# muzishen/IMAGDressing

Measured on NVIDIA H100. Metric: images/sec, 512x512 50-step DDIM garment-conditioned (CFG), higher is better.
Workload: dtype bf16

## Files before the change

### imagdressing_b200/_lib.py

```python
from __future__ import annotations

import ctypes
import os
from ctypes import POINTER, Structure, c_char_p, c_float, c_int, c_int32, c_int64, c_void_p

_HERE = os.path.dirname(os.path.abspath(__file__))
LIB_PATH = os.path.join(_HERE, "libimagd_b200.so")

IMAGD_OK = 0
ACT_NONE, ACT_GEGLU, ACT_SILU, ACT_GELU, ACT_QUICK_GELU = 0, 1, 2, 3, 4


class Epilogue(Structure):

    _fields_ = [
        ("bias", c_void_p),
        ("rowvec", c_void_p),
        ("rowvec_ld", c_int64),
        ("rows_per_group", c_int32),
        ("act", c_int32),
        ("residual", c_void_p),
        ("ldr", c_int64),
        ("alpha", c_float),
        ("out_fp32", c_int32),
        ("row_stats_out", c_void_p),
        ("stats_ld", c_int64),
        ("row_stats_in", c_void_p),
        ("stats_in_ld", c_int64),
        ("stats_parts", c_int32),
        ("ln_dim", c_int32),
        ("ln_eps", c_float),
        ("colsum", c_void_p),
    ]


class AttnTrain(Structure):

    _fields_ = [("lse", c_void_p), ("out_s0", c_void_p), ("out_s1", c_void_p), ("ld_s", c_int64), ("lq_pad", c_int32)]


class KVStream(Structure):

    _fields_ = [
        ("k", c_void_p),
        ("v", c_void_p),
        ("ld", c_int64),
        ("len", c_int32),
        ("sample_rows", c_int32),
        ("broadcast", c_int32),
        ("n_query_samples", c_int32),
        ("out_scale", c_float),
    ]


SIGNATURES = {
    "imagd_version": (c_int, []),
    "imagd_last_error": (c_char_p, []),
    "imagd_device_check": (c_int, []),
    "imagd_gemm_bf16": (c_int, [c_void_p, c_int64, c_void_p, c_int64, c_void_p, c_int64, c_int, c_int, c_int,
                                POINTER(Epilogue), c_void_p]),
    "imagd_gemm_debug_force": (c_int, [c_int, c_int, c_int]),
    "imagd_gemm_debug_log": (c_int, [c_int, c_char_p, c_int]),
    "imagd_gemm_debug_timeline": (c_int, [c_void_p]),
    "imagd_gemm_tile_count_n": (c_int, [c_int, c_int, c_int]),
    "imagd_conv3x3_bf16": (c_int, [c_void_p, c_int64, c_int, c_int, c_int, c_int, c_void_p, c_void_p, c_int64, c_int,
                                   POINTER(Epilogue), c_void_p]),
    "imagd_upconv3x3_bf16": (c_int, [c_void_p, c_int64, c_int, c_int, c_int, c_int, c_void_p, c_void_p, c_int64, c_int,
                                     POINTER(Epilogue), c_void_p]),
    "imagd_attention_bf16": (c_int, [c_void_p, c_int64, c_void_p, c_int64, c_int, c_int, c_int, c_int,
                                     POINTER(KVStream), POINTER(KVStream), c_float, c_void_p]),
    "imagd_attention_causal_bf16": (c_int, [c_void_p, c_int64, c_void_p, c_int64, c_int, c_int, c_int, c_int,
                                            POINTER(KVStream), c_float, c_void_p]),
    "imagd_groupnorm_ws_bytes": (c_int64, [c_int, c_int, c_int, c_int]),
    "imagd_groupnorm_bf16": (c_int, [c_void_p, c_int64, c_void_p, c_int64, c_int, c_int, c_int, c_int, c_void_p,
                                     c_void_p, c_float, c_int, c_void_p, c_void_p]),
    "imagd_layernorm_bf16": (c_int, [c_void_p, c_int64, c_void_p, c_int64, c_int, c_int, c_void_p, c_void_p, c_float,
                                     c_void_p]),
    "imagd_concat_add_bf16": (c_int, [c_void_p, c_int64, c_int, c_void_p, c_int64, c_void_p, c_int64, c_int, c_void_p,
                                      c_int64, c_void_p, c_int64, c_int64, c_void_p]),
    "imagd_upsample2x_bf16": (c_int, [c_void_p, c_void_p, c_int, c_int, c_int, c_int, c_void_p]),
    "imagd_im2col3x3_s2_bf16": (c_int, [c_void_p, c_void_p, c_int, c_int, c_int, c_int, c_void_p]),
    "imagd_im2col3x3_s2_pad_bf16": (c_int, [c_void_p, c_void_p, c_int, c_int, c_int, c_int, c_int, c_void_p]),
    "imagd_embed_tokens_bf16": (c_int, [c_void_p, c_void_p, c_void_p, c_void_p, c_int, c_int, c_int, c_int, c_void_p]),
    "imagd_patchify_bf16": (c_int, [c_void_p, c_void_p, c_int, c_int, c_int, c_int, c_int, c_void_p]),
    "imagd_broadcast_row_bf16": (c_int, [c_void_p, c_void_p, c_int, c_int64, c_int, c_int, c_void_p]),
    "imagd_softmax_rows": (c_int, [c_void_p, c_int64, c_void_p, c_int64, c_int64, c_int, c_float, c_void_p]),
    "imagd_conv3x3_direct_bf16": (c_int, [c_void_p, c_int, c_int, c_int, c_int, c_void_p, c_void_p, c_void_p, c_int,
                                          c_int, c_int, c_int, c_void_p, c_void_p]),
    "imagd_nchw_f32_to_nhwc_bf16": (c_int, [c_void_p, c_void_p, c_int, c_int, c_int, c_int, c_int, c_int, c_void_p]),
    "imagd_timestep_embedding": (c_int, [c_void_p, c_void_p, c_void_p, c_int, c_int, c_void_p]),
    "imagd_linear_small_m": (c_int, [c_void_p, c_int64, c_void_p, c_int64, c_void_p, c_void_p, c_int64, c_int, c_int,
                                     c_int, c_int, c_int, c_void_p]),
    "imagd_cfg_ddim_step": (c_int, [c_void_p, c_void_p, c_float, c_void_p, c_void_p, c_void_p, c_void_p, c_void_p,
                                    c_void_p, c_void_p, c_int, c_int, c_int, c_void_p]),
    "imagd_nchw_f32_to_nhwc_bf16_scaled": (c_int, [c_void_p, c_void_p, c_int, c_int, c_int, c_int, c_int, c_int, c_void_p,
                                                   c_void_p, c_void_p]),
    "imagd_cfg_sampler_step": (c_int, [c_void_p, c_void_p, c_float, c_void_p, c_void_p, c_void_p, c_void_p, c_void_p,
                                       c_void_p, c_void_p, c_void_p, c_void_p, c_int, c_int, c_int, c_void_p]),
    "imagd_attention_train_fwd_bf16": (c_int, [c_void_p, c_int64, c_void_p, c_int64, c_int, c_int, c_int, c_int,
                                               POINTER(KVStream), POINTER(KVStream), c_float, POINTER(AttnTrain), c_void_p]),
    "imagd_attention_bwd_prep": (c_int, [c_void_p, c_int64, c_void_p, c_void_p, c_int64, c_float, c_float, c_void_p, c_int,
                                         c_int, c_int, c_int, c_int, c_void_p]),
    "imagd_attention_bwd_bf16": (c_int, [c_void_p, c_int64, c_void_p, c_int64, c_int, c_int, c_int, c_int, POINTER(KVStream),
                                         POINTER(KVStream), c_float, c_void_p, c_void_p, c_int, c_void_p, c_int64, c_void_p,
                                         c_void_p, c_int64, c_void_p, c_void_p, c_int64, c_void_p]),
    "imagd_transpose_bf16": (c_int, [c_void_p, c_int64, c_void_p, c_int64, c_int, c_int, c_int, c_void_p]),
    "imagd_conv_weight_layout_bf16": (c_int, [c_void_p, c_void_p, c_int, c_int, c_int, c_void_p]),
    "imagd_conv_weight_flip_bf16": (c_int, [c_void_p, c_void_p, c_int, c_int, c_void_p]),
    "imagd_im2col3x3_t_bf16": (c_int, [c_void_p, c_void_p, c_int64, c_int, c_int, c_int, c_int, c_void_p]),
    "imagd_col2im3x3_s2_bf16": (c_int, [c_void_p, c_void_p, c_int, c_int, c_int, c_int, c_void_p]),
    "imagd_downsum2x_bf16": (c_int, [c_void_p, c_void_p, c_int, c_int, c_int, c_int, c_void_p]),
    "imagd_colreduce_ws_bytes": (c_int64, [c_int, c_int, c_int]),
    "imagd_colsum_bf16": (c_int, [c_void_p, c_int64, c_int, c_int, c_int, c_void_p, c_int, c_void_p, c_void_p]),
    "imagd_layernorm_bwd_bf16": (c_int, [c_void_p, c_int64, c_void_p, c_int64, c_void_p, c_int64, c_int, c_int, c_void_p,
                                         c_float, c_void_p, c_void_p, c_int, c_void_p, c_void_p, c_void_p]),
    "imagd_groupnorm_stats_bf16": (c_int, [c_void_p, c_int64, c_void_p, c_int64, c_int, c_int, c_int, c_int, c_void_p,
                                           c_void_p, c_float, c_int, c_void_p, c_void_p, c_void_p]),
    "imagd_groupnorm_bwd_ws_bytes": (c_int64, [c_int, c_int, c_int, c_int]),
    "imagd_groupnorm_bwd_bf16": (c_int, [c_void_p, c_void_p, c_void_p, c_int, c_int, c_int, c_int, c_void_p, c_void_p,
                                         c_void_p, c_int, c_void_p, c_void_p, c_int, c_void_p, c_void_p]),
    "imagd_act_bf16": (c_int, [c_void_p, c_void_p, c_void_p, c_int64, c_int, c_void_p]),
    "imagd_geglu_bf16": (c_int, [c_void_p, c_int64, c_void_p, c_void_p, c_int64, c_int64, c_int, c_void_p]),
    "imagd_mse_loss_grad": (c_int, [c_void_p, c_void_p, c_void_p, c_void_p, c_int64, c_float, c_void_p, c_void_p]),
    "imagd_adamw_step": (c_int, [c_void_p, c_void_p, c_void_p, c_void_p, c_void_p, c_int64, c_float, c_float, c_float,
                                 c_float, c_float, c_int, c_float, c_void_p]),
    "imagd_adamw_step_dev": (c_int, [c_void_p, c_void_p, c_void_p, c_void_p, c_void_p, c_int64, c_float, c_float, c_float,
# ... 102 lines not shown
```

### imagdressing_b200/csrc/norm.cu

```cuda
#include <cooperative_groups.h>

#include <cstdlib>

#include "common.cuh"
#include "ptx.cuh"

namespace imagd {

constexpr int kGnMaxC = 2560;
constexpr int kGnThreads = 512;
constexpr int kGnCounters = 1024;

static int gn_pixels_per_chunk() {
    static int v = 0;
    if (v == 0) {
        const char* e = getenv("IMAGD_GN_PX");
        v = e ? atoi(e) : 16;
        if (v < 4 || v > 256) v = 16;
    }
    return v;
}
static int gn_max_chunks() {
    static int v = 0;
    if (v == 0) {
        const char* e = getenv("IMAGD_GN_MAXCHUNKS");
        v = e ? atoi(e) : 64;
        if (v < 1 || v > kNumSms) v = 64;
    }
    return v;
}
inline int gn_chunks(int HW, int NB) {
    const int px = gn_pixels_per_chunk();
    int c = (HW + px - 1) / px;
    const int cap = (kNumSms * 2) / (NB > 0 ? NB : 1);
    if (c > gn_max_chunks()) c = gn_max_chunks();
    if (c > cap) c = cap;
    return c < 1 ? 1 : c;
}

__global__ void __launch_bounds__(kGnThreads, 2) groupnorm_fused_kernel(
    const __nv_bfloat16* __restrict__ x, int64_t ldx, __nv_bfloat16* __restrict__ y, int64_t ldy, int HW, int C,
    int groups, int chunks, float* __restrict__ ws, const float* __restrict__ gamma, const float* __restrict__ beta,
    float eps, int fuse_silu, float* __restrict__ stats_out) {
    pdl_launch_dependents();
    pdl_wait();
    __shared__ float s_a[kGnThreads * 8];
    __shared__ float s_b[kGnThreads * 8];
    __shared__ float s_mean[64];
    __shared__ float s_rstd[64];
    extern __shared__ float s_affine[];
    float* s_gamma = s_affine;
    float* s_beta = s_affine + C;
    float* s_piv = s_affine + 2 * C;
    const int n = blockIdx.y, chunk = blockIdx.x;
    const int CV = C / 8;
    const int rows = kGnThreads / CV;
    const int ppc = (HW + chunks - 1) / chunks;
    const int p_begin = chunk * ppc;
    const int p_end = min(HW, p_begin + ppc);
    const int cpg = C / groups;
    for (int c = threadIdx.x; c < C; c += kGnThreads) {
        s_gamma[c] = gamma ? __ldg(gamma + c) : 1.f;
        s_beta[c] = beta ? __ldg(beta + c) : 0.f;
    }
    unsigned int* counters = reinterpret_cast<unsigned int*>(ws) - kGnCounters + 2 * n;

    const int cv = threadIdx.x % CV;
    const int prow = threadIdx.x / CV;
    if (prow < rows) {
        float sum[8], sq[8], piv[8];
#pragma unroll
        for (int k = 0; k < 8; ++k) sum[k] = sq[k] = piv[k] = 0.f;
        const __nv_bfloat16* base = x + (static_cast<int64_t>(n) * HW) * ldx + cv * 8;
        if (p_begin < p_end) {
            const uint4 pv = __ldg(reinterpret_cast<const uint4*>(base + static_cast<int64_t>(p_begin) * ldx));
            const uint32_t u[4] = {pv.x, pv.y, pv.z, pv.w};
#pragma unroll
            for (int k = 0; k < 4; ++k) {
                piv[2 * k] = bf16lo(u[k]);
                piv[2 * k + 1] = bf16hi(u[k]);
            }
        }
        if (prow == 0) {
#pragma unroll
            for (int k = 0; k < 8; ++k) s_piv[cv * 8 + k] = piv[k];
        }
        for (int pix = p_begin + prow; pix < p_end; pix += rows * 4) {
            uint4 v[4];
// ... 108 lines not shown
        }
        __syncthreads();
    }
    for (int c = threadIdx.x; c < C; c += kGnThreads) {
        const int g = c / cpg;
        const float sc = s_gamma[c] * s_rstd[g];
        s_a[c] = sc;
        s_b[c] = s_beta[c] - s_mean[g] * sc;
    }
    __syncthreads();
    const int total = (p_end - p_begin) * CV;
    constexpr int U = 4;
    const int step_row = kGnThreads / CV, step_col = kGnThreads % CV;
    int walk_row = threadIdx.x / CV, walk_col = threadIdx.x % CV;
    for (int base = threadIdx.x; base < total; base += kGnThreads * U) {
        uint4 v[U];
        int c0s[U];
        int64_t rowsv[U];
#pragma unroll
        for (int t = 0; t < U; ++t) {
            const int idx = base + t * kGnThreads;
            v[t] = make_uint4(0u, 0u, 0u, 0u);
            c0s[t] = walk_col * 8;
            rowsv[t] = static_cast<int64_t>(n) * HW + p_begin + walk_row;
            if (idx < total) v[t] = __ldg(reinterpret_cast<const uint4*>(x + rowsv[t] * ldx + c0s[t]));
            walk_row += step_row;
            walk_col += step_col;
            if (walk_col >= CV) {
                walk_col -= CV;
                ++walk_row;
            }
        }
#pragma unroll
        for (int t = 0; t < U; ++t) {
            if (base + t * kGnThreads >= total) break;
            const uint32_t u[4] = {v[t].x, v[t].y, v[t].z, v[t].w};
            const int c0 = c0s[t];
            float f[8];
#pragma unroll
            for (int k = 0; k < 4; ++k) {
                f[2 * k] = bf16lo(u[k]) * s_a[c0 + 2 * k] + s_b[c0 + 2 * k];
                f[2 * k + 1] = bf16hi(u[k]) * s_a[c0 + 2 * k + 1] + s_b[c0 + 2 * k + 1];
            }
            if (fuse_silu) {
#pragma unroll
                for (int k = 0; k < 8; ++k) f[k] = silu(f[k]);
            }
            *reinterpret_cast<uint4*>(y + rowsv[t] * ldy + c0) = make_uint4(
                pack_bf16x2(f[0], f[1]), pack_bf16x2(f[2], f[3]), pack_bf16x2(f[4], f[5]), pack_bf16x2(f[6], f[7]));
        }
    }
}

constexpr int kGnCS = 8;
__global__ void __launch_bounds__(kGnThreads, 2) groupnorm_cluster_kernel(
    const __nv_bfloat16* __restrict__ x, int64_t ldx, __nv_bfloat16* __restrict__ y, int64_t ldy, int HW, int C,
    int groups, int gps, const float* __restrict__ gamma, const float* __restrict__ beta, float eps, int fuse_silu,
    float* __restrict__ stats_out) {
    pdl_launch_dependents();
    pdl_wait();
    namespace cg = cooperative_groups;
    cg::cluster_group cluster = cg::this_cluster();
    __shared__ float s_a[kGnThreads * 8];
    __shared__ float s_b[kGnThreads * 8];
    __shared__ float s_part[64 * 2];
    __shared__ float s_mean[64];
    __shared__ float s_rstd[64];
    extern __shared__ __align__(16) unsigned char s_dyn[];
    const int cpg = C / groups;
    const int SC = gps * cpg;
    const int SV = SC / 8;
    float* s_gamma = reinterpret_cast<float*>(s_dyn);
    float* s_beta = s_gamma + SC;
    float* s_piv = s_beta + SC;
    uint4* tile = reinterpret_cast<uint4*>(s_dyn + ((3 * SC * sizeof(float) + 15) / 16) * 16);
    const int rank = static_cast<int>(cluster.block_rank());
    const int slice = blockIdx.x / kGnCS, n = blockIdx.y;
    const int c_base = slice * SC;
    const int rpc = (HW + kGnCS - 1) / kGnCS;
    const int p_begin = min(HW, rank * rpc);
    const int p_end = min(HW, p_begin + rpc);
    for (int c = threadIdx.x; c < SC; c += kGnThreads) {
        s_gamma[c] = gamma ? __ldg(gamma + c_base + c) : 1.f;
        s_beta[c] = beta ? __ldg(beta + c_base + c) : 0.f;
    }
    const int cv = threadIdx.x % SV;
    const int prow = threadIdx.x / SV;
    const int rows = kGnThreads / SV;
    if (prow < rows) {
        float sum[8], sq[8], piv[8];
#pragma unroll
        for (int k = 0; k < 8; ++k) sum[k] = sq[k] = piv[k] = 0.f;
        const __nv_bfloat16* base = x + (static_cast<int64_t>(n) * HW) * ldx + c_base + cv * 8;
        if (p_begin < p_end) {
            const uint4 pv = __ldg(reinterpret_cast<const uint4*>(base + static_cast<int64_t>(p_begin) * ldx));
            const uint32_t u[4] = {pv.x, pv.y, pv.z, pv.w};
#pragma unroll
            for (int k = 0; k < 4; ++k) {
                piv[2 * k] = bf16lo(u[k]);
                piv[2 * k + 1] = bf16hi(u[k]);
            }
        }
        if (prow == 0) {
#pragma unroll
            for (int k = 0; k < 8; ++k) s_piv[cv * 8 + k] = piv[k];
        }
        for (int pix = p_begin + prow; pix < p_end; pix += rows * 4) {
            uint4 v[4];
            float live[4];
#pragma unroll
            for (int t = 0; t < 4; ++t) {
                v[t] = make_uint4(0u, 0u, 0u, 0u);
                live[t] = 0.f;
                if (pix + t * rows < p_end) {
                    v[t] = __ldg(reinterpret_cast<const uint4*>(base + static_cast<int64_t>(pix + t * rows) * ldx));
                    live[t] = 1.f;
                }
            }
#pragma unroll
            for (int t = 0; t < 4; ++t) {
                if (pix + t * rows < p_end) tile[(pix + t * rows - p_begin) * SV + cv] = v[t];
                const uint32_t u[4] = {v[t].x, v[t].y, v[t].z, v[t].w};
#pragma unroll
                for (int k = 0; k < 4; ++k) {
                    const float a = (bf16lo(u[k]) - piv[2 * k]) * live[t], b = (bf16hi(u[k]) - piv[2 * k + 1]) * live[t];
                    sum[2 * k] += a;
                    sq[2 * k] += a * a;
                    sum[2 * k + 1] += b;
                    sq[2 * k + 1] += b * b;
                }
            }
        }
#pragma unroll
        for (int k = 0; k < 8; ++k) {
            s_a[prow * SC + cv * 8 + k] = sum[k];
            s_b[prow * SC + cv * 8 + k] = sq[k];
        }
    }
    __syncthreads();
    for (int c = threadIdx.x; c < SC; c += kGnThreads) {
        float a = s_a[c], b = s_b[c];
        for (int r = 1; r < rows; ++r) {
            a += s_a[r * SC + c];
            b += s_b[r * SC + c];
        }
        s_a[c] = a;
        s_b[c] = b;
    }
    __syncthreads();
    if (threadIdx.x < gps) {
        const int g = threadIdx.x;
        const float npix = static_cast<float>(p_end - p_begin);
        const float inv = npix > 0.f ? 1.f / npix : 0.f;
        float mean_g = 0.f;
        for (int c = g * cpg; c < (g + 1) * cpg; ++c) mean_g += s_piv[c] + s_a[c] * inv;
        mean_g /= static_cast<float>(cpg);
        float m2 = 0.f;
        for (int c = g * cpg; c < (g + 1) * cpg; ++c) {
            const float d = s_piv[c] + s_a[c] * inv - mean_g;
            m2 += (s_b[c] - s_a[c] * s_a[c] * inv) + npix * d * d;
        }
        s_part[2 * g] = npix > 0.f ? mean_g : 0.f;
        s_part[2 * g + 1] = npix > 0.f ? m2 : 0.f;
    }
    cluster.sync();
    if (threadIdx.x < gps) {
        const int g = threadIdx.x;
        float a = 0.f, b = 0.f;
        const float pivot = cluster.map_shared_rank(s_part, 0)[2 * g];
        for (int r = 0; r < kGnCS; ++r) {
            const float* rp = cluster.map_shared_rank(s_part, r);
            const float cnt_r = static_cast<float>(cpg) * static_cast<float>(max(min(HW, (r + 1) * rpc) - min(HW, r * rpc), 0));
            const float d = rp[2 * g] - pivot;
            a += cnt_r * d;
            b += rp[2 * g + 1] + cnt_r * d * d;
        }
        const float cnt = static_cast<float>(cpg) * static_cast<float>(HW);
        const float dm = a / cnt;
        const float var = fmaxf((b - a * dm) / cnt, 0.f);
        s_mean[g] = pivot + dm;
        s_rstd[g] = rsqrtf(var + eps);
        if (stats_out != nullptr && rank == 0) {
            stats_out[(static_cast<int64_t>(n) * groups + slice * gps + g) * 2] = pivot + dm;
            stats_out[(static_cast<int64_t>(n) * groups + slice * gps + g) * 2 + 1] = s_rstd[g];
        }
    }
    cluster.barrier_arrive();
    __syncthreads();
    for (int c = threadIdx.x; c < SC; c += kGnThreads) {
        const int g = c / cpg;
        const float sc = s_gamma[c] * s_rstd[g];
        s_a[c] = sc;
        s_b[c] = s_beta[c] - s_mean[g] * sc;
    }
    __syncthreads();
    const int total = (p_end - p_begin) * SV;
    const int step_row = kGnThreads / SV, step_col = kGnThreads % SV;
    int walk_row = prow, walk_col = cv;
    for (int idx = threadIdx.x; idx < total; idx += kGnThreads) {
        const uint4 v = tile[idx];
        const int c0 = walk_col * 8;
        const int64_t row = static_cast<int64_t>(n) * HW + p_begin + walk_row;
        walk_row += step_row;
        walk_col += step_col;
        if (walk_col >= SV) {
            walk_col -= SV;
            ++walk_row;
        }
        const uint32_t u[4] = {v.x, v.y, v.z, v.w};
        float f[8];
#pragma unroll
        for (int k = 0; k < 4; ++k) {
            f[2 * k] = bf16lo(u[k]) * s_a[c0 + 2 * k] + s_b[c0 + 2 * k];
            f[2 * k + 1] = bf16hi(u[k]) * s_a[c0 + 2 * k + 1] + s_b[c0 + 2 * k + 1];
        }
        if (fuse_silu) {
#pragma unroll
            for (int k = 0; k < 8; ++k) f[k] = silu(f[k]);
        }
        *reinterpret_cast<uint4*>(y + row * ldy + c_base + c0) = make_uint4(
            pack_bf16x2(f[0], f[1]), pack_bf16x2(f[2], f[3]), pack_bf16x2(f[4], f[5]), pack_bf16x2(f[6], f[7]));
    }
    cluster.barrier_wait();
}

template <int VPL, int R>
__global__ void __launch_bounds__(256) layernorm_kernel(const __nv_bfloat16* __restrict__ x, int64_t ldx,
                                                        __nv_bfloat16* __restrict__ y, int64_t ldy, int rows, int C,
// ... 30 lines not shown
                f[i][2 * k] = bf16lo(u[k]);
                f[i][2 * k + 1] = bf16hi(u[k]);
                sum += f[i][2 * k] + f[i][2 * k + 1];
            }
        }
#pragma unroll
        for (int o = 16; o > 0; o >>= 1) sum += __shfl_xor_sync(0xffffffffu, sum, o);
        const float mean = sum * inv_c;
        float sq = 0.f;
#pragma unroll
        for (int i = 0; i < VPL; ++i) {
            if (lane + i * 32 < CV) {
#pragma unroll
                for (int k = 0; k < 8; ++k) {
                    const float d = f[i][k] - mean;
                    sq += d * d;
                }
            }
        }
#pragma unroll
        for (int o = 16; o > 0; o >>= 1) sq += __shfl_xor_sync(0xffffffffu, sq, o);
        const float rstd = rsqrtf(sq * inv_c + eps);
#pragma unroll
        for (int i = 0; i < VPL; ++i) {
            const int cv = lane + i * 32;
            if (cv < CV) {
                float o[8];
                float g[8], b[8];
                if (gamma) {
                    const float4 g0 = __ldg(reinterpret_cast<const float4*>(gamma + cv * 8));
                    const float4 g1 = __ldg(reinterpret_cast<const float4*>(gamma + cv * 8 + 4));
                    g[0] = g0.x; g[1] = g0.y; g[2] = g0.z; g[3] = g0.w; g[4] = g1.x; g[5] = g1.y; g[6] = g1.z; g[7] = g1.w;
                } else {
#pragma unroll
                    for (int k = 0; k < 8; ++k) g[k] = 1.f;
                }
                if (beta) {
                    const float4 b0 = __ldg(reinterpret_cast<const float4*>(beta + cv * 8));
                    const float4 b1 = __ldg(reinterpret_cast<const float4*>(beta + cv * 8 + 4));
                    b[0] = b0.x; b[1] = b0.y; b[2] = b0.z; b[3] = b0.w; b[4] = b1.x; b[5] = b1.y; b[6] = b1.z; b[7] = b1.w;
                } else {
#pragma unroll
                    for (int k = 0; k < 8; ++k) b[k] = 0.f;
                }
#pragma unroll
                for (int k = 0; k < 8; ++k) o[k] = (f[i][k] - mean) * rstd * g[k] + b[k];
                *reinterpret_cast<uint4*>(y + static_cast<int64_t>(row0 + r) * ldy + cv * 8) =
                    make_uint4(pack_bf16x2(o[0], o[1]), pack_bf16x2(o[2], o[3]), pack_bf16x2(o[4], o[5]), pack_bf16x2(o[6], o[7]));
            }
        }
    }
}

static int gn_cluster_mode() {
    static int v = -1;
    if (v < 0) {
        const char* e = getenv("IMAGD_GN_CLUSTER");
        v = e ? atoi(e) : 1;
        if (v < 0 || v > 2) v = 1;
    }
    return v;
}
struct GnClusterPlan {
    int gps;
    size_t smem;
};
constexpr size_t kGnClusterMaxDyn = 190 * 1024;
static bool gn_cluster_plan(int NB, int HW, int C, int groups, GnClusterPlan* plan) {
    const int mode = gn_cluster_mode();
    if (mode == 0) return false;
    const int cpg = C / groups;
    if (mode == 1 && cpg < 10) return false;
    const int rpc = (HW + kGnCS - 1) / kGnCS;
    double best = 0.0;
    bool found = false;
    for (int gps = 1; gps <= groups; ++gps) {
        if (groups % gps != 0) continue;
        const int SC = gps * cpg;
        if (SC % 8 != 0 || SC / 8 > kGnThreads) continue;
        const size_t tile = static_cast<size_t>(rpc) * SC * 2;
        const size_t dyn = (3 * static_cast<size_t>(SC) * sizeof(float) + 15) / 16 * 16 + tile;
        if (dyn > kGnClusterMaxDyn) continue;
        const int per_sm = (dyn + 35 * 1024) * 2 <= 228 * 1024 ? 2 : 1;
        const int64_t ctas = static_cast<int64_t>(NB) * (groups / gps) * kGnCS;
        const int64_t slots = 144LL * per_sm;
        const int64_t waves = (ctas + slots - 1) / slots;
        if (mode == 1 && (waves > 1 || tile > 32 * 1024)) continue;
        const double cost = static_cast<double>(waves) * (64.0 * 1024 + static_cast<double>(tile) * (SC * 2 < 128 ? 1.3 : 1.0));
        if (!found || cost < best) {
            best = cost;
            plan->gps = gps;
            plan->smem = dyn;
            found = true;
        }
    }
    return found;
}

template <int VPL, int R>
static int launch_ln(const void* x, int64_t ldx, void* y, int64_t ldy, int rows, int C, const float* gamma,
                     const float* beta, float eps, cudaStream_t st) {
    const int rows_per_block = 8 * R;
    IMAGD_CUDA(launch_pdl(layernorm_kernel<VPL, R>, dim3((rows + rows_per_block - 1) / rows_per_block), dim3(256), 0, st,
                          reinterpret_cast<const __nv_bfloat16*>(x), ldx, reinterpret_cast<__nv_bfloat16*>(y), ldy, rows, C,
                          gamma, beta, eps));
    return IMAGD_OK;
}

}

extern "C" {

int64_t imagd_groupnorm_ws_bytes(int NB, int HW, int C, int groups) {
    (void)C;
    return (imagd::kGnCounters + static_cast<int64_t>(NB) * imagd::gn_chunks(HW, NB) * groups * 2) * sizeof(float);
}

int imagd_groupnorm_bf16(const void* x, int64_t ldx, void* y, int64_t ldy, int NB, int HW, int C, int groups,
                         const float* gamma, const float* beta, float eps, int fuse_silu, void* ws, imagd_stream stream) {
    return imagd_groupnorm_stats_bf16(x, ldx, y, ldy, NB, HW, C, groups, gamma, beta, eps, fuse_silu, ws, nullptr, stream);
}

int imagd_groupnorm_stats_bf16(const void* x, int64_t ldx, void* y, int64_t ldy, int NB, int HW, int C, int groups,
                               const float* gamma, const float* beta, float eps, int fuse_silu, void* ws, float* stats_out,
                               imagd_stream stream) {
    using namespace imagd;
    IMAGD_CHECK_ARG(x && y && ws, "groupnorm: null pointer");
    IMAGD_CHECK_ARG(NB > 0 && 2 * NB <= kGnCounters && NB <= kNumSms * 2 && HW > 0 && C > 0 && C % 8 == 0 && C <= kGnMaxC,
                    "groupnorm: NB=%d C=%d unsupported", NB, C);
    IMAGD_CHECK_ARG(groups > 0 && groups <= 64 && C % groups == 0, "groupnorm: groups=%d", groups);
    IMAGD_CHECK_ARG(ldx % 8 == 0 && ldy % 8 == 0 && aligned16(x) && aligned16(y), "groupnorm: alignment");
    cudaStream_t st = static_cast<cudaStream_t>(stream);
    GnClusterPlan plan;
    if (gn_cluster_plan(NB, HW, C, groups, &plan)) {
        IMAGD_SET_MAX_SMEM(groupnorm_cluster_kernel, static_cast<int>(kGnClusterMaxDyn));
        cudaLaunchConfig_t cfg{};
        cfg.gridDim = dim3(kGnCS * (groups / plan.gps), NB);
        cfg.blockDim = dim3(kGnThreads);
        cfg.dynamicSmemBytes = plan.smem;
        cfg.stream = st;
        cudaLaunchAttribute attr[2];
        attr[0].id = cudaLaunchAttributeClusterDimension;
        attr[0].val.clusterDim.x = kGnCS;
        attr[0].val.clusterDim.y = 1;
        attr[0].val.clusterDim.z = 1;
        attr[1].id = cudaLaunchAttributeProgrammaticStreamSerialization;
        attr[1].val.programmaticStreamSerializationAllowed = 1;
        cfg.attrs = attr;
        cfg.numAttrs = pdl_enabled() ? 2 : 1;
        IMAGD_CUDA(cudaLaunchKernelEx(&cfg, groupnorm_cluster_kernel, reinterpret_cast<const __nv_bfloat16*>(x), ldx,
                                      reinterpret_cast<__nv_bfloat16*>(y), ldy, HW, C, groups, plan.gps, gamma, beta, eps,
                                      fuse_silu, stats_out));
        return IMAGD_OK;
    }
    const int chunks = gn_chunks(HW, NB);
    IMAGD_SET_MAX_SMEM(groupnorm_fused_kernel, 64 * 1024);
    IMAGD_CUDA(launch_pdl(groupnorm_fused_kernel, dim3(chunks, NB), dim3(kGnThreads), 3 * C * sizeof(float), st,
                          reinterpret_cast<const __nv_bfloat16*>(x), ldx, reinterpret_cast<__nv_bfloat16*>(y), ldy, HW, C,
                          groups, chunks, reinterpret_cast<float*>(ws) + kGnCounters, gamma, beta, eps, fuse_silu, stats_out));
    return IMAGD_OK;
}

int imagd_layernorm_bf16(const void* x, int64_t ldx, void* y, int64_t ldy, int rows, int C, const float* gamma,
                         const float* beta, float eps, imagd_stream stream) {
    using namespace imagd;
    IMAGD_CHECK_ARG(x && y, "layernorm: null pointer");
    IMAGD_CHECK_ARG(rows > 0 && C > 0 && C % 8 == 0 && C <= 2048, "layernorm: C=%d unsupported", C);
    IMAGD_CHECK_ARG(ldx % 8 == 0 && ldy % 8 == 0 && aligned16(x) && aligned16(y), "layernorm: alignment");
    IMAGD_CHECK_ARG((!gamma || aligned16(gamma)) && (!beta || aligned16(beta)), "layernorm: gamma/beta alignment");
    cudaStream_t st = static_cast<cudaStream_t>(stream);
    const int vpl = (C / 8 + 31) / 32;
    if (vpl <= 2) return launch_ln<2, 4>(x, ldx, y, ldy, rows, C, gamma, beta, eps, st);
    if (vpl <= 3) return launch_ln<3, 4>(x, ldx, y, ldy, rows, C, gamma, beta, eps, st);
    if (vpl <= 5) return launch_ln<5, 2>(x, ldx, y, ldy, rows, C, gamma, beta, eps, st);
    return launch_ln<8, 1>(x, ldx, y, ldy, rows, C, gamma, beta, eps, st);

}

}
```

### include/imagd_b200.h

```cpp
#ifndef IMAGD_B200_H
#define IMAGD_B200_H

#include <stdint.h>

#ifdef __cplusplus
extern "C" {
#endif

typedef void* imagd_stream;

enum imagd_status {
    IMAGD_OK = 0,
    IMAGD_ERR_ARG = -1,
    IMAGD_ERR_CUDA = -2,
    IMAGD_ERR_ARCH = -3
};

enum imagd_act { IMAGD_ACT_NONE = 0, IMAGD_ACT_GEGLU = 1, IMAGD_ACT_SILU = 2, IMAGD_ACT_GELU = 3,
                 IMAGD_ACT_QUICK_GELU = 4  };

int imagd_version(void);
const char* imagd_last_error(void);
int imagd_device_check(void);

// ... 1 lines not shown
    const float* bias;
    const float* rowvec;
    int64_t rowvec_ld;
    int32_t rows_per_group;
    int32_t act;
    const void* residual;
    int64_t ldr;
    float alpha;
    int32_t out_fp32;
    float* row_stats_out;
    int64_t stats_ld;
    const float* row_stats_in;
    int64_t stats_in_ld;
    int32_t stats_parts;
    int32_t ln_dim;
    float ln_eps;
    const float* colsum;
} imagd_epilogue;

int imagd_gemm_bf16(const void* A, int64_t lda, const void* W, int64_t ldw, void* D, int64_t ldd, int M, int N,
                    int K, const imagd_epilogue* ep, imagd_stream stream);

int imagd_gemm_debug_force(int block_n, int stages, int splits);
int imagd_upconv3x3_bf16(const void* X, int64_t ldx, int NB, int H, int W, int Cin, const void* Wt, void* Y, int64_t ldy,
                         int Cout, const imagd_epilogue* ep, imagd_stream stream);
int imagd_gemm_tile_count_n(int M, int N, int K);
int imagd_gemm_debug_log(int enable, char* out, int out_bytes);
int imagd_gemm_debug_timeline(void* device_buf);

int imagd_conv3x3_bf16(const void* X, int64_t ldx, int NB, int H, int W, int Cin, const void* Wt, void* Y,
                       int64_t ldy, int Cout, const imagd_epilogue* ep, imagd_stream stream);

typedef struct imagd_kv_stream {
    const void* k;
    const void* v;
    int64_t ld;
    int32_t len;
    int32_t sample_rows;
    int32_t broadcast;
    int32_t n_query_samples;
    float out_scale;
} imagd_kv_stream;

int imagd_attention_bf16(const void* q, int64_t q_ld, void* out, int64_t out_ld, int B, int Lq, int heads,
                         int head_dim, const imagd_kv_stream* s0, const imagd_kv_stream* s1, float sm_scale,
                         imagd_stream stream);
int imagd_attention_causal_bf16(const void* q, int64_t q_ld, void* out, int64_t out_ld, int B, int Lq, int heads,
                                int head_dim, const imagd_kv_stream* s0, float sm_scale, imagd_stream stream);

int64_t imagd_groupnorm_ws_bytes(int NB, int HW, int C, int groups);
int imagd_groupnorm_bf16(const void* x, int64_t ldx, void* y, int64_t ldy, int NB, int HW, int C, int groups,
                         const float* gamma, const float* beta, float eps, int fuse_silu, void* ws,
                         imagd_stream stream);
int imagd_layernorm_bf16(const void* x, int64_t ldx, void* y, int64_t ldy, int rows, int C, const float* gamma,
                         const float* beta, float eps, imagd_stream stream);

int imagd_concat_add_bf16(const void* a, int64_t lda, int Ca, const void* res_a, int64_t ld_ra, const void* b,
                          int64_t ldb, int Cb, const void* res_b, int64_t ld_rb, void* out, int64_t ldo,
                          int64_t rows, imagd_stream stream);
int imagd_upsample2x_bf16(const void* x, void* y, int NB, int H, int W, int C, imagd_stream stream);
int imagd_im2col3x3_s2_bf16(const void* x, void* col, int NB, int H, int W, int C, imagd_stream stream);
int imagd_im2col3x3_s2_pad_bf16(const void* x, void* col, int NB, int H, int W, int C, int pad_lo, imagd_stream stream);
int imagd_softmax_rows(const float* s, int64_t lds, void* p, int64_t ldp, int64_t rows, int cols, float scale,
                       imagd_stream stream);
int imagd_conv3x3_direct_bf16(const void* x, int NB, int H, int W, int Cin, const void* w, const float* bias,
                              void* y, int Cout, int stride, int act, int out_nchw_f32, const void* add_nhwc,
                              imagd_stream stream);
int imagd_nchw_f32_to_nhwc_bf16(const float* x, void* y, int NB, int C, int H, int W, int Cpad, int repeat,
                                imagd_stream stream);
int imagd_nchw_f32_to_nhwc_bf16_scaled(const float* x, void* y, int NB, int C, int H, int W, int Cpad, int repeat,
                                       const float* scale_table, const int32_t* step_ptr, imagd_stream stream);

int imagd_embed_tokens_bf16(const int64_t* ids, const void* tok, const void* pos, void* out, int rows, int T, int C, int vocab,
                            imagd_stream stream);
int imagd_patchify_bf16(const float* x, void* out, int B, int H, int W, int patch, int Kpad, imagd_stream stream);
int imagd_broadcast_row_bf16(const void* vec, void* out, int B, int64_t rows_per_sample, int row, int C, imagd_stream stream);

int imagd_timestep_embedding(const float* timesteps, const int32_t* step_ptr, float* out, int NB, int dim,
                             imagd_stream stream);
int imagd_linear_small_m(const float* x, int64_t ldx, const void* W, int64_t ldw, const float* bias, float* out,
                         int64_t ldo, int M, int N, int K, int act_in, int act_out, imagd_stream stream);

int imagd_cfg_ddim_step(const float* eps_cond, const float* eps_uncond, float guidance, float* latents,
                        const float* coef, int32_t* step_ptr, const float* mask, const float* image_latents,
                        const float* noise, const float* blend_coef, int NB, int C, int HW,
                        imagd_stream stream);
int imagd_cfg_sampler_step(const float* eps_cond, const float* eps_uncond, float guidance, float* latents,
                           float* history, const float* step_noise, const float* coef, int32_t* step_ptr,
                           const float* mask, const float* image_latents, const float* noise, const float* blend_coef,
                           int NB, int C, int HW, imagd_stream stream);


typedef struct imagd_attn_train {
    float* lse;
    void* out_s0;
    void* out_s1;
    int64_t ld_s;
    int32_t lq_pad;
} imagd_attn_train;

int imagd_attention_train_fwd_bf16(const void* q, int64_t q_ld, void* out, int64_t out_ld, int B, int Lq, int heads,
                                   int head_dim, const imagd_kv_stream* s0, const imagd_kv_stream* s1, float sm_scale,
                                   const imagd_attn_train* aux, imagd_stream stream);
int imagd_attention_bwd_prep(const void* d_out, int64_t do_ld, const void* o0, const void* o1, int64_t ld_s, float w0, float w1,
                             float* dsum, int B, int Lq, int heads, int head_dim, int lq_pad, imagd_stream stream);
int imagd_attention_bwd_bf16(const void* q, int64_t q_ld, const void* d_out, int64_t do_ld, int B, int Lq, int heads,
// ... 39 lines not shown
```

Before: 2.700.

## Add cost-model planner choosing groupnorm cluster size and slice width

The groupnorm launcher now picks among cluster sizes 2/4/8/16 and channel-slice widths using queried cluster occupancy and a fitted cost model, falling back to the rendezvous kernel when that model predicts it is cheaper. The cluster kernel is templated on cluster size, reduces its per-row partial sums in parallel, and reads remote DSMEM partials as vectorised float2 loads. Environment-variable tuning knobs are removed, and plan-query, force and log debug entry points are added. The aim is better SM utilisation and shorter reductions for groupnorm across the UNet's shapes. The cost model's constants were fitted on a particular GPU and may pick poorly on others, and the capacity query adds one-time setup work.

Measured after the change: 2.806 (median of 6 runs). 1.04x the previous value.

```diff
diff --git a/imagdressing_b200/_lib.py b/imagdressing_b200/_lib.py
--- a/imagdressing_b200/_lib.py
+++ b/imagdressing_b200/_lib.py
@@ -72,6 +72,10 @@
     "imagd_attention_causal_bf16": (c_int, [c_void_p, c_int64, c_void_p, c_int64, c_int, c_int, c_int, c_int,
                                             POINTER(KVStream), c_float, c_void_p]),
     "imagd_groupnorm_ws_bytes": (c_int64, [c_int, c_int, c_int, c_int]),
+    "imagd_groupnorm_plan": (c_int, [c_int, c_int, c_int, c_int, c_void_p, c_void_p]),
+    "imagd_groupnorm_cluster_capacity": (c_int, [c_void_p]),
+    "imagd_groupnorm_debug_force": (c_int, [c_int, c_int, c_int]),
+    "imagd_groupnorm_debug_log": (c_int, [c_int, c_char_p, c_int]),
     "imagd_groupnorm_bf16": (c_int, [c_void_p, c_int64, c_void_p, c_int64, c_int, c_int, c_int, c_int, c_void_p,
                                      c_void_p, c_float, c_int, c_void_p, c_void_p]),
     "imagd_layernorm_bf16": (c_int, [c_void_p, c_int64, c_void_p, c_int64, c_int, c_int, c_void_p, c_void_p, c_float,
diff --git a/imagdressing_b200/csrc/norm.cu b/imagdressing_b200/csrc/norm.cu
--- a/imagdressing_b200/csrc/norm.cu
+++ b/imagdressing_b200/csrc/norm.cu
@@ -1,6 +1,12 @@
 #include <cooperative_groups.h>
 
-#include <cstdlib>
+#include <algorithm>
+#include <cstdio>
+#include <cstring>
+#include <mutex>
+#include <string>
+#include <utility>
+#include <vector>
 
 #include "common.cuh"
 #include "ptx.cuh"
@@ -11,29 +17,10 @@
 constexpr int kGnThreads = 512;
 constexpr int kGnCounters = 1024;
 
-static int gn_pixels_per_chunk() {
-    static int v = 0;
-    if (v == 0) {
-        const char* e = getenv("IMAGD_GN_PX");
-        v = e ? atoi(e) : 16;
-        if (v < 4 || v > 256) v = 16;
-    }
-    return v;
-}
-static int gn_max_chunks() {
-    static int v = 0;
-    if (v == 0) {
-        const char* e = getenv("IMAGD_GN_MAXCHUNKS");
-        v = e ? atoi(e) : 64;
-        if (v < 1 || v > kNumSms) v = 64;
-    }
-    return v;
-}
 inline int gn_chunks(int HW, int NB) {
-    const int px = gn_pixels_per_chunk();
-    int c = (HW + px - 1) / px;
+    int c = (HW + 15) / 16;
     const int cap = (kNumSms * 2) / (NB > 0 ? NB : 1);
-    if (c > gn_max_chunks()) c = gn_max_chunks();
+    if (c > 64) c = 64;
     if (c > cap) c = cap;
     return c < 1 ? 1 : c;
 }
@@ -248,7 +235,7 @@
     }
 }
 
-constexpr int kGnCS = 8;
+template <int CS>
 __global__ void __launch_bounds__(kGnThreads, 2) groupnorm_cluster_kernel(
     const __nv_bfloat16* __restrict__ x, int64_t ldx, __nv_bfloat16* __restrict__ y, int64_t ldy, int HW, int C,
     int groups, int gps, const float* __restrict__ gamma, const float* __restrict__ beta, float eps, int fuse_silu,
@@ -259,7 +246,7 @@
     cg::cluster_group cluster = cg::this_cluster();
     __shared__ float s_a[kGnThreads * 8];
     __shared__ float s_b[kGnThreads * 8];
-    __shared__ float s_part[64 * 2];
+    __shared__ __align__(8) float s_part[64 * 2];
     __shared__ float s_mean[64];
     __shared__ float s_rstd[64];
     extern __shared__ __align__(16) unsigned char s_dyn[];
@@ -271,9 +258,9 @@
     float* s_piv = s_beta + SC;
     uint4* tile = reinterpret_cast<uint4*>(s_dyn + ((3 * SC * sizeof(float) + 15) / 16) * 16);
     const int rank = static_cast<int>(cluster.block_rank());
-    const int slice = blockIdx.x / kGnCS, n = blockIdx.y;
+    const int slice = blockIdx.x / CS, n = blockIdx.y;
     const int c_base = slice * SC;
-    const int rpc = (HW + kGnCS - 1) / kGnCS;
+    const int rpc = (HW + CS - 1) / CS;
     const int p_begin = min(HW, rank * rpc);
     const int p_end = min(HW, p_begin + rpc);
     for (int c = threadIdx.x; c < SC; c += kGnThreads) {
@@ -303,23 +290,20 @@
         }
         for (int pix = p_begin + prow; pix < p_end; pix += rows * 4) {
             uint4 v[4];
-            float live[4];
 #pragma unroll
             for (int t = 0; t < 4; ++t) {
                 v[t] = make_uint4(0u, 0u, 0u, 0u);
-                live[t] = 0.f;
-                if (pix + t * rows < p_end) {
+                if (pix + t * rows < p_end)
                     v[t] = __ldg(reinterpret_cast<const uint4*>(base + static_cast<int64_t>(pix + t * rows) * ldx));
-                    live[t] = 1.f;
-                }
             }
 #pragma unroll
             for (int t = 0; t < 4; ++t) {
-                if (pix + t * rows < p_end) tile[(pix + t * rows - p_begin) * SV + cv] = v[t];
+                if (pix + t * rows >= p_end) break;
+                tile[(pix + t * rows - p_begin) * SV + cv] = v[t];
                 const uint32_t u[4] = {v[t].x, v[t].y, v[t].z, v[t].w};
 #pragma unroll
                 for (int k = 0; k < 4; ++k) {
-                    const float a = (bf16lo(u[k]) - piv[2 * k]) * live[t], b = (bf16hi(u[k]) - piv[2 * k + 1]) * live[t];
+                    const float a = bf16lo(u[k]) - piv[2 * k], b = bf16hi(u[k]) - piv[2 * k + 1];
                     sum[2 * k] += a;
                     sq[2 * k] += a * a;
                     sum[2 * k + 1] += b;
@@ -334,11 +318,23 @@
         }
     }
     __syncthreads();
+    const int parts = max(1, min(rows, kGnThreads / SC));
+    for (int idx = threadIdx.x; idx < SC * parts; idx += kGnThreads) {
+        const int c = idx % SC, p = idx / SC;
+        float a = s_a[p * SC + c], b = s_b[p * SC + c];
+        for (int r = p + parts; r < rows; r += parts) {
+            a += s_a[r * SC + c];
+            b += s_b[r * SC + c];
+        }
+        s_a[p * SC + c] = a;
+        s_b[p * SC + c] = b;
+    }
+    __syncthreads();
     for (int c = threadIdx.x; c < SC; c += kGnThreads) {
         float a = s_a[c], b = s_b[c];
-        for (int r = 1; r < rows; ++r) {
-            a += s_a[r * SC + c];
-            b += s_b[r * SC + c];
+        for (int p = 1; p < parts; ++p) {
+            a += s_a[p * SC + c];
+            b += s_b[p * SC + c];
         }
         s_a[c] = a;
         s_b[c] = b;
@@ -363,13 +359,16 @@
     if (threadIdx.x < gps) {
         const int g = threadIdx.x;
         float a = 0.f, b = 0.f;
-        const float pivot = cluster.map_shared_rank(s_part, 0)[2 * g];
-        for (int r = 0; r < kGnCS; ++r) {
-            const float* rp = cluster.map_shared_rank(s_part, r);
+        float2 part[CS];
+#pragma unroll
+        for (int r = 0; r < CS; ++r) part[r] = reinterpret_cast<const float2*>(cluster.map_shared_rank(s_part, r))[g];
+        const float pivot = part[0].x;
+#pragma unroll
+        for (int r = 0; r < CS; ++r) {
             const float cnt_r = static_cast<float>(cpg) * static_cast<float>(max(min(HW, (r + 1) * rpc) - min(HW, r * rpc), 0));
-            const float d = rp[2 * g] - pivot;
+            const float d = part[r].x - pivot;
             a += cnt_r * d;
-            b += rp[2 * g + 1] + cnt_r * d * d;
+            b += part[r].y + cnt_r * d * d;
         }
         const float cnt = static_cast<float>(cpg) * static_cast<float>(HW);
         const float dm = a / cnt;
@@ -506,49 +505,118 @@
     }
 }
 
-static int gn_cluster_mode() {
-    static int v = -1;
-    if (v < 0) {
-        const char* e = getenv("IMAGD_GN_CLUSTER");
-        v = e ? atoi(e) : 1;
-        if (v < 0 || v > 2) v = 1;
-    }
-    return v;
-}
-struct GnClusterPlan {
-    int gps;
-    size_t smem;
+constexpr int kGnClusterSizes[4] = {2, 4, 8, 16};
+constexpr size_t kGnClusterMaxDyn = 190 * 1024;
+constexpr size_t kGnTwoPerSmDyn = 76 * 1024;
+enum { kGnAuto = 0, kGnRendezvous = 1, kGnCluster = 2 };
+struct GnPlan {
+    int kernel;
+    int cs;
+    int sc;
+    int smem;
+    int waves;
 };
-constexpr size_t kGnClusterMaxDyn = 190 * 1024;
-static bool gn_cluster_plan(int NB, int HW, int C, int groups, GnClusterPlan* plan) {
-    const int mode = gn_cluster_mode();
-    if (mode == 0) return false;
+static int g_gn_force[3] = {0, 0, 0};
+static int g_gn_log_on = 0;
+static std::vector<std::pair<std::string, int>> g_gn_log;
+static std::mutex g_gn_mutex;
+
+template <int CS>
+static cudaError_t gn_cluster_launch(const cudaLaunchConfig_t* cfg, const __nv_bfloat16* x, int64_t ldx, __nv_bfloat16* y,
+                                     int64_t ldy, int HW, int C, int groups, int gps, const float* gamma, const float* beta,
+                                     float eps, int fuse_silu, float* stats_out) {
+    return cudaLaunchKernelEx(cfg, groupnorm_cluster_kernel<CS>, x, ldx, y, ldy, HW, C, groups, gps, gamma, beta, eps,
+                              fuse_silu, stats_out);
+}
+
+template <int CS>
+static int gn_query_capacity(size_t dyn) {
+    if (cudaFuncSetAttribute(groupnorm_cluster_kernel<CS>, cudaFuncAttributeMaxDynamicSharedMemorySize,
+                             static_cast<int>(kGnClusterMaxDyn)) != cudaSuccess ||
+        (CS > 8 && cudaFuncSetAttribute(groupnorm_cluster_kernel<CS>, cudaFuncAttributeNonPortableClusterSizeAllowed, 1) !=
+                       cudaSuccess)) {
+        cudaGetLastError();
+        return 0;
+    }
+    cudaLaunchConfig_t cfg{};
+    cfg.gridDim = dim3(CS);
+    cfg.blockDim = dim3(kGnThreads);
+    cfg.dynamicSmemBytes = dyn;
+    cudaLaunchAttribute attr;
+    attr.id = cudaLaunchAttributeClusterDimension;
+    attr.val.clusterDim.x = CS;
+    attr.val.clusterDim.y = attr.val.clusterDim.z = 1;
+    cfg.attrs = &attr;
+    cfg.numAttrs = 1;
+    int n = 0;
+    if (cudaOccupancyMaxActiveClusters(&n, groupnorm_cluster_kernel<CS>, &cfg) != cudaSuccess) {
+        cudaGetLastError();
+        return 0;
+    }
+    return n;
+}
+static int gn_device_capacity(int* cap) {
+    static int cache[16][8];
+    static bool have[16];
+    int dev = 0;
+    IMAGD_CUDA(cudaGetDevice(&dev));
+    IMAGD_CHECK_ARG(dev >= 0 && dev < 16, "groupnorm: device index %d", dev);
+    std::lock_guard<std::mutex> lock(g_gn_mutex);
+    if (!have[dev]) {
+        const size_t dyn[2] = {kGnClusterMaxDyn, kGnTwoPerSmDyn};
+        for (int k = 0; k < 2; ++k) {
+            cache[dev][0 + k] = gn_query_capacity<2>(dyn[k]);
+            cache[dev][2 + k] = gn_query_capacity<4>(dyn[k]);
+            cache[dev][4 + k] = gn_query_capacity<8>(dyn[k]);
+            cache[dev][6 + k] = gn_query_capacity<16>(dyn[k]);
+        }
+        have[dev] = true;
+    }
+    memcpy(cap, cache[dev], sizeof(cache[dev]));
+    return IMAGD_OK;
+}
+
+static double gn_cluster_cost(double mb, int smem, bool two_per_sm) {
+    return 6.32 + 0.0715 * (smem / 1024.0) * (two_per_sm ? 2.0 : 1.0) + 0.0194 * mb + (two_per_sm ? 0.98 : 0.0);
+}
+static double gn_rendezvous_cost(double mb, int C) {
+    return 8.23 + 0.291 * std::min(mb, 40.0) + 0.608 * std::max(mb - 40.0, 0.0) + 2.17 * (C / 1024.0) + (C >= 2560 ? 4.72 : 0.0);
+}
+
+static bool gn_plan(int NB, int HW, int C, int groups, const int* cap, GnPlan* plan) {
     const int cpg = C / groups;
-    if (mode == 1 && cpg < 10) return false;
-    const int rpc = (HW + kGnCS - 1) / kGnCS;
+    const double mb = 4.0 * NB * HW * C / 1e6;
+    const bool forced_cluster = g_gn_force[0] == kGnCluster || g_gn_force[1] || g_gn_force[2];
     double best = 0.0;
     bool found = false;
-    for (int gps = 1; gps <= groups; ++gps) {
-        if (groups % gps != 0) continue;
-        const int SC = gps * cpg;
-        if (SC % 8 != 0 || SC / 8 > kGnThreads) continue;
-        const size_t tile = static_cast<size_t>(rpc) * SC * 2;
-        const size_t dyn = (3 * static_cast<size_t>(SC) * sizeof(float) + 15) / 16 * 16 + tile;
-        if (dyn > kGnClusterMaxDyn) continue;
-        const int per_sm = (dyn + 35 * 1024) * 2 <= 228 * 1024 ? 2 : 1;
-        const int64_t ctas = static_cast<int64_t>(NB) * (groups / gps) * kGnCS;
-        const int64_t slots = 144LL * per_sm;
-        const int64_t waves = (ctas + slots - 1) / slots;
-        if (mode == 1 && (waves > 1 || tile > 32 * 1024)) continue;
-        const double cost = static_cast<double>(waves) * (64.0 * 1024 + static_cast<double>(tile) * (SC * 2 < 128 ? 1.3 : 1.0));
-        if (!found || cost < best) {
-            best = cost;
-            plan->gps = gps;
-            plan->smem = dyn;
-            found = true;
-        }
-    }
-    return found;
+    for (int i = 0; i < 4 && g_gn_force[0] != kGnRendezvous; ++i) {
+        const int cs = kGnClusterSizes[i];
+        if (g_gn_force[1] && g_gn_force[1] != cs) continue;
+        const int rpc = (HW + cs - 1) / cs;
+        for (int gps = 1; gps <= groups; ++gps) {
+            const int sc = gps * cpg;
+            if (groups % gps != 0 || sc % 8 != 0 || (g_gn_force[2] && g_gn_force[2] != sc)) continue;
+            const size_t tile = static_cast<size_t>(rpc) * sc * 2;
+            const size_t dyn = (3 * static_cast<size_t>(sc) * sizeof(float) + 15) / 16 * 16 + tile;
+            if (dyn > kGnClusterMaxDyn) continue;
+            const int64_t clusters = static_cast<int64_t>(NB) * (groups / gps);
+            const bool two_per_sm = clusters > cap[2 * i] && dyn <= kGnTwoPerSmDyn;
+            const int slots = cap[2 * i + (two_per_sm ? 1 : 0)];
+            if (slots <= 0) continue;
+            const int waves = static_cast<int>((clusters + slots - 1) / slots);
+            if (waves > 1 && !forced_cluster) continue;
+            const double cost = waves * gn_cluster_cost(mb, static_cast<int>(dyn), two_per_sm);
+            if (!found || cost < best) {
+                best = cost;
+                *plan = GnPlan{kGnCluster, cs, sc, static_cast<int>(dyn), waves};
+                found = true;
+            }
+        }
+    }
+    if (forced_cluster) return found;
+    if (found && g_gn_force[0] == kGnAuto && best <= gn_rendezvous_cost(mb, C)) return true;
+    *plan = GnPlan{kGnRendezvous, 0, 0, static_cast<int>(3 * C * sizeof(float)), 1};
+    return true;
 }
 
 template <int VPL, int R>
@@ -585,34 +653,105 @@
     IMAGD_CHECK_ARG(groups > 0 && groups <= 64 && C % groups == 0, "groupnorm: groups=%d", groups);
     IMAGD_CHECK_ARG(ldx % 8 == 0 && ldy % 8 == 0 && aligned16(x) && aligned16(y), "groupnorm: alignment");
     cudaStream_t st = static_cast<cudaStream_t>(stream);
-    GnClusterPlan plan;
-    if (gn_cluster_plan(NB, HW, C, groups, &plan)) {
-        IMAGD_SET_MAX_SMEM(groupnorm_cluster_kernel, static_cast<int>(kGnClusterMaxDyn));
+    int cap[8];
+    int rc = gn_device_capacity(cap);
+    if (rc != IMAGD_OK) return rc;
+    GnPlan plan;
+    IMAGD_CHECK_ARG(gn_plan(NB, HW, C, groups, cap, &plan), "groupnorm: no legal plan for the forced kernel %d cluster %d slice %d",
+                    g_gn_force[0], g_gn_force[1], g_gn_force[2]);
+    if (g_gn_log_on) {
+        char key[128];
+        snprintf(key, sizeof(key), "%d %d %d %d | %d %d %d %d %d", NB, HW, C, groups, plan.kernel, plan.cs, plan.sc, plan.smem,
+                 plan.waves);
+        std::lock_guard<std::mutex> lock(g_gn_mutex);
+        auto it = std::find_if(g_gn_log.begin(), g_gn_log.end(), [&](const auto& e) { return e.first == key; });
+        if (it == g_gn_log.end()) g_gn_log.emplace_back(key, 1);
+        else ++it->second;
+    }
+    const __nv_bfloat16* xb = reinterpret_cast<const __nv_bfloat16*>(x);
+    __nv_bfloat16* yb = reinterpret_cast<__nv_bfloat16*>(y);
+    if (plan.kernel == kGnCluster) {
         cudaLaunchConfig_t cfg{};
-        cfg.gridDim = dim3(kGnCS * (groups / plan.gps), NB);
+        cfg.gridDim = dim3(plan.cs * (C / plan.sc), NB);
         cfg.blockDim = dim3(kGnThreads);
         cfg.dynamicSmemBytes = plan.smem;
         cfg.stream = st;
         cudaLaunchAttribute attr[2];
         attr[0].id = cudaLaunchAttributeClusterDimension;
-        attr[0].val.clusterDim.x = kGnCS;
+        attr[0].val.clusterDim.x = plan.cs;
         attr[0].val.clusterDim.y = 1;
         attr[0].val.clusterDim.z = 1;
         attr[1].id = cudaLaunchAttributeProgrammaticStreamSerialization;
         attr[1].val.programmaticStreamSerializationAllowed = 1;
         cfg.attrs = attr;
         cfg.numAttrs = pdl_enabled() ? 2 : 1;
-        IMAGD_CUDA(cudaLaunchKernelEx(&cfg, groupnorm_cluster_kernel, reinterpret_cast<const __nv_bfloat16*>(x), ldx,
-                                      reinterpret_cast<__nv_bfloat16*>(y), ldy, HW, C, groups, plan.gps, gamma, beta, eps,
-                                      fuse_silu, stats_out));
+        const int gps = plan.sc / (C / groups);
+        switch (plan.cs) {
+            case 2: IMAGD_CUDA(gn_cluster_launch<2>(&cfg, xb, ldx, yb, ldy, HW, C, groups, gps, gamma, beta, eps, fuse_silu, stats_out)); break;
+            case 4: IMAGD_CUDA(gn_cluster_launch<4>(&cfg, xb, ldx, yb, ldy, HW, C, groups, gps, gamma, beta, eps, fuse_silu, stats_out)); break;
+            case 8: IMAGD_CUDA(gn_cluster_launch<8>(&cfg, xb, ldx, yb, ldy, HW, C, groups, gps, gamma, beta, eps, fuse_silu, stats_out)); break;
+            default: IMAGD_CUDA(gn_cluster_launch<16>(&cfg, xb, ldx, yb, ldy, HW, C, groups, gps, gamma, beta, eps, fuse_silu, stats_out)); break;
+        }
         return IMAGD_OK;
     }
     const int chunks = gn_chunks(HW, NB);
     IMAGD_SET_MAX_SMEM(groupnorm_fused_kernel, 64 * 1024);
-    IMAGD_CUDA(launch_pdl(groupnorm_fused_kernel, dim3(chunks, NB), dim3(kGnThreads), 3 * C * sizeof(float), st,
-                          reinterpret_cast<const __nv_bfloat16*>(x), ldx, reinterpret_cast<__nv_bfloat16*>(y), ldy, HW, C,
+    IMAGD_CUDA(launch_pdl(groupnorm_fused_kernel, dim3(chunks, NB), dim3(kGnThreads), plan.smem, st, xb, ldx, yb, ldy, HW, C,
                           groups, chunks, reinterpret_cast<float*>(ws) + kGnCounters, gamma, beta, eps, fuse_silu, stats_out));
     return IMAGD_OK;
+}
+
+int imagd_groupnorm_plan(int NB, int HW, int C, int groups, const int* cluster_capacity, int* out) {
+    using namespace imagd;
+    IMAGD_CHECK_ARG(out && NB > 0 && HW > 0 && C > 0 && C % 8 == 0 && C <= kGnMaxC && groups > 0 && groups <= 64 &&
+                        C % groups == 0,
+                    "groupnorm_plan: NB=%d HW=%d C=%d groups=%d", NB, HW, C, groups);
+    int cap[8];
+    if (cluster_capacity) {
+        memcpy(cap, cluster_capacity, sizeof(cap));
+    } else {
+        int rc = gn_device_capacity(cap);
+        if (rc != IMAGD_OK) return rc;
+    }
+    GnPlan plan;
+    IMAGD_CHECK_ARG(gn_plan(NB, HW, C, groups, cap, &plan), "groupnorm_plan: no legal plan for the forced kernel %d cluster %d slice %d",
+                    g_gn_force[0], g_gn_force[1], g_gn_force[2]);
+    const int v[5] = {plan.kernel, plan.cs, plan.sc, plan.smem, plan.waves};
+    memcpy(out, v, sizeof(v));
+    return IMAGD_OK;
+}
+
+int imagd_groupnorm_cluster_capacity(int* out) {
+    IMAGD_CHECK_ARG(out, "groupnorm_cluster_capacity: null pointer");
+    return imagd::gn_device_capacity(out);
+}
+
+int imagd_groupnorm_debug_force(int kernel, int cluster_size, int slice_channels) {
+    IMAGD_CHECK_ARG(kernel >= 0 && kernel <= 2 && (kernel != imagd::kGnRendezvous || (!cluster_size && !slice_channels)),
+                    "groupnorm_debug_force: kernel %d", kernel);
+    IMAGD_CHECK_ARG(cluster_size == 0 || cluster_size == 2 || cluster_size == 4 || cluster_size == 8 || cluster_size == 16,
+                    "groupnorm_debug_force: cluster size %d", cluster_size);
+    IMAGD_CHECK_ARG(slice_channels >= 0 && slice_channels % 8 == 0, "groupnorm_debug_force: slice of %d channels", slice_channels);
+    imagd::g_gn_force[0] = kernel;
+    imagd::g_gn_force[1] = cluster_size;
+    imagd::g_gn_force[2] = slice_channels;
+    return IMAGD_OK;
+}
+
+int imagd_groupnorm_debug_log(int enable, char* out, int out_bytes) {
+    std::lock_guard<std::mutex> lock(imagd::g_gn_mutex);
+    if (enable >= 0) {
+        imagd::g_gn_log_on = enable;
+        if (enable) imagd::g_gn_log.clear();
+    }
+    if (out && out_bytes > 0) {
+        std::string all;
+        for (const auto& k : imagd::g_gn_log) all += k.first + " | " + std::to_string(k.second) + "\n";
+        IMAGD_CHECK_ARG(static_cast<int>(all.size()) < out_bytes, "groupnorm_debug_log: buffer too small (%d needed)",
+                        static_cast<int>(all.size()) + 1);
+        memcpy(out, all.c_str(), all.size() + 1);
+    }
+    return static_cast<int>(imagd::g_gn_log.size());
 }
 
 int imagd_layernorm_bf16(const void* x, int64_t ldx, void* y, int64_t ldy, int rows, int C, const float* gamma,
diff --git a/include/imagd_b200.h b/include/imagd_b200.h
--- a/include/imagd_b200.h
+++ b/include/imagd_b200.h
@@ -77,6 +77,10 @@
 int imagd_groupnorm_bf16(const void* x, int64_t ldx, void* y, int64_t ldy, int NB, int HW, int C, int groups,
                          const float* gamma, const float* beta, float eps, int fuse_silu, void* ws,
                          imagd_stream stream);
+int imagd_groupnorm_plan(int NB, int HW, int C, int groups, const int* cluster_capacity, int* out);
+int imagd_groupnorm_cluster_capacity(int* out);
+int imagd_groupnorm_debug_force(int kernel, int cluster_size, int slice_channels);
+int imagd_groupnorm_debug_log(int enable, char* out, int out_bytes);
 int imagd_layernorm_bf16(const void* x, int64_t ldx, void* y, int64_t ldy, int rows, int C, const float* gamma,
                          const float* beta, float eps, imagd_stream stream);
 
```
